# hkust-vgd/scanobjectnn

Hardware: NVIDIA H100
Metric: point-clouds/sec (B=32, N=2048, 15-class) (higher is better)
Workload: dtype f32

## Files before the change

scanobjectnn_b200/csrc/mlp.cu:

```cuda
#include <float.h>

#include "common.cuh"
#include "mlp_internal.cuh"

namespace psa {

constexpr int kMlpThreads = 256;
constexpr int BM = 128;
constexpr int BK = 16;
constexpr int BN_MAX = 128;

__device__ __forceinline__ void cp_async16(void* smem_dst, const void* gmem_src) {
    unsigned d = (unsigned)__cvta_generic_to_shared(smem_dst);
    asm volatile("cp.async.cg.shared.global [%0], [%1], 16;\n" ::"r"(d), "l"(gmem_src));
}
__device__ __forceinline__ void cp_async_commit() { asm volatile("cp.async.commit_group;\n" ::); }
template <int N>
__device__ __forceinline__ void cp_async_wait() {
    asm volatile("cp.async.wait_group %0;\n" ::"n"(N));
}

__device__ __forceinline__ int f2ord(float f) {
    int i = __float_as_int(f);
    return i >= 0 ? i : i ^ 0x7fffffff;
// ... 335 lines not shown
}

template <int TN>
__global__ void __launch_bounds__(kMlpThreads, 2)
dense_layer_kernel(const __grid_constant__ DenseArgs a) {
    constexpr int BN = 16 * TN;
    __shared__ __align__(16) float As[2][BM * LDA_D];
    __shared__ __align__(16) float Ws[2][BK * BN];
    __shared__ int s_pool[(TN == 8) ? 16 * BN : 32 * BN];
    const int tid = threadIdx.x;
    const int ty = tid >> 4, tx = tid & 15;
    const long long row0 = (long long)blockIdx.x * BM;
    const int n0 = blockIdx.y * BN;
    const int K4 = (a.K + 3) & ~3;
    const int nchunks = (K4 + BK - 1) / BK;
    float acc[8][TN];
#pragma unroll
    for (int i = 0; i < 8; ++i)
#pragma unroll
        for (int j = 0; j < TN; ++j) acc[i][j] = 0.f;
    load_a_chunk(As[0], a.x, row0, a.rows, a.K, 0, tid);
    load_w_chunk<BN>(Ws[0], a.W, a.K, a.N, 0, n0, -1, tid);
    cp_async_commit();
    for (int c = 0; c < nchunks; ++c) {
        if (c + 1 < nchunks) {
            load_a_chunk(As[(c + 1) & 1], a.x, row0, a.rows, a.K, (c + 1) * BK, tid);
            load_w_chunk<BN>(Ws[(c + 1) & 1], a.W, a.K, a.N, (c + 1) * BK, n0, -1, tid);
            cp_async_commit();
            cp_async_wait<1>();
        } else {
            cp_async_wait<0>();
        }
        __syncthreads();
        mma_chunk<TN>(As[c & 1], LDA_D, Ws[c & 1], min(BK, K4 - c * BK), acc, ty, tx);
        __syncthreads();
    }
    const int tile_rows = (int)min((long long)BM, a.rows - row0);
    const int pk = a.pool_k;
    if (a.group_add != nullptr) {
#pragma unroll
        for (int i = 0; i < 8; ++i) {
            const int row = ty * 8 + i;
            if (row >= tile_rows) break;
            const float* ga = a.group_add + (row0 + row) / a.group_rows * a.N;
#pragma unroll
            for (int h = 0; h < TN / 4; ++h)
#pragma unroll
                for (int j = 0; j < 4; ++j) {
                    const int col = n0 + h * 64 + tx * 4 + j;
                    if (col < a.N) acc[i][h * 4 + j] += __ldg(ga + col);
                }
        }
    }
    if (pk == 1) {
#pragma unroll
        for (int h = 0; h < TN / 4; ++h) {
            const int col = n0 + h * 64 + tx * 4;
#pragma unroll
            for (int j = 0; j < 4; ++j) {
                if (col + j >= a.N) continue;
                const float sc = a.scale ? __ldg(a.scale + col + j) : 1.f;
                const float sh = a.shift ? __ldg(a.shift + col + j) : 0.f;
#pragma unroll
                for (int i = 0; i < 8; ++i) {
                    const int row = ty * 8 + i;
                    if (row < tile_rows) {
                        float v = fmaf(acc[i][h * 4 + j], sc, sh);
                        if (a.relu) v = fmaxf(v, 0.f);
                        a.out[(row0 + row) * a.N + col + j] = v;
                    }
                }
            }
        }
        return;
    }
    const bool inside = pk <= BM;
    const int ngroups = inside ? (tile_rows / pk) : 1;
    for (int s = tid; s < ngroups * BN; s += kMlpThreads) s_pool[s] = f2ord(__int_as_float(0xff800000));
    __syncthreads();
#pragma unroll
    for (int h = 0; h < TN / 4; ++h) {
        const int col = n0 + h * 64 + tx * 4;
#pragma unroll
        for (int j = 0; j < 4; ++j) {
            if (col + j >= a.N) continue;
            const float sc = a.scale ? __ldg(a.scale + col + j) : 1.f;
            const float sh = a.shift ? __ldg(a.shift + col + j) : 0.f;
            int curg = -1;
            float m = 0.f;
#pragma unroll
            for (int i = 0; i < 8; ++i) {
                const int row = ty * 8 + i;
                if (row >= tile_rows) break;
                float v = fmaf(acc[i][h * 4 + j], sc, sh);
                if (a.relu) v = fmaxf(v, 0.f);
                const int g = inside ? row / pk : 0;
                if (g != curg) {
                    if (curg >= 0) atomicMax(&s_pool[curg * BN + h * 64 + tx * 4 + j], f2ord(m));
                    curg = g;
                    m = v;
                } else {
                    m = fmaxf(m, v);
                }
            }
            if (curg >= 0) atomicMax(&s_pool[curg * BN + h * 64 + tx * 4 + j], f2ord(m));
        }
// ... 199 lines not shown
```

scanobjectnn_b200/csrc/mlp_internal.cuh:

```cuda
#pragma once
#include "common.cuh"

namespace psa {

struct DenseArgs {
    long long rows;
    int K, N;
    int pool_k;
    int relu;
    const float* x;
    const float* W;
    const float* scale;
    const float* shift;
    float* out;
    const float* group_add = nullptr;
    long long group_rows = 0;
};


int launch_dense(const DenseArgs& d, cudaStream_t st);
size_t fc_small_workspace_bytes(int K, int N);
int launch_fc_small(const DenseArgs& d, float* partial, cudaStream_t st);
int sa_module_simt(int b, int n, int m, int c, int nsample, const float* xyz, const float* new_xyz, const float* points,
                   const int* idx, const psa_mlp* mlp, float* out, cudaStream_t st);
int validate_mlp_public(const psa_mlp* mlp, const char* who);
int edgeconv_simt(int b, int n, int c, int k, const float* x, const int* nn_idx, const psa_mlp* mlp, float* out, cudaStream_t st);
int launch_fill_ord_neg_inf(long long total, float* out, cudaStream_t st, const unsigned int* run_if = nullptr);
int launch_decode_ord(long long total, float* out, cudaStream_t st, const unsigned int* run_if = nullptr);
size_t edge_tail_workspace_bytes(int b, int n, int c, int k, int N);
int edge_layer_tail(int b, int n, int c, int k, int N, const float* x, const int* nn_idx, const float* W, const float* PQ, const float* scale,
                    const float* shift, const float* coef, const float* pooled, const float* R, const float* dz, float* dW, float* dx,
                    void* workspace, cudaStream_t st);
int frozen_coef(int N, const float* scale, float* coef, cudaStream_t st);

int mlp_mode();
int tc_np();
int tc_dense_nt(long long rows, int N);
int build_image(int K, int Kp, int N, int Nt, const float* W, uint8_t* image, cudaStream_t st, const unsigned int* run_if = nullptr);
const unsigned int* image_trailer(const uint8_t* image, int Kp, int N);
const float* image_colscale(const uint8_t* image, int Kp, int N);

}

__global__ void edge_wc_kernel(int c, int N, const float* __restrict__ W, float* __restrict__ Wc);
```

scanobjectnn_b200/csrc/tc_mlp.cu:

```cuda
#include <float.h>
#include <stdlib.h>

#include <algorithm>
#include <atomic>
#include <type_traits>

#include "common.cuh"
#include "mlp_internal.cuh"
#include "ring_gemm.cuh"
#include "tc_common.cuh"

namespace psa {

using namespace tc;

constexpr int kMaxTcLayers = 2;


struct TcArgs {
    long long groups;
    int K;
    int n, m;
    const float* xyz;
    const float* new_xyz;
// ... 69 lines not shown
    s_bad[threadIdx.y][threadIdx.x] = bad;
    __syncthreads();
    if (threadIdx.y != 0 || n >= N) return;
    for (int y = 1; y < 8; ++y) { m = fmaxf(m, s_max[y][threadIdx.x]); bad = bad || s_bad[y][threadIdx.x]; }
    int e = 0;
    if (!bad && m > 0.f) e = min(137 - (int)(__float_as_uint(m) >> 23), 64);
    colscale[n] = __int_as_float((127 - e) << 23);
    if (bad) atomicOr(trailer, 1u);
}

template <int NP>
__global__ void tc_prep_weights_kernel(int K, int Kp, int N, int Nt, const float* __restrict__ W, const float* __restrict__ colscale,
                                       uint8_t* __restrict__ image, const unsigned int* __restrict__ run_if) {
    if (run_if != nullptr && *run_if == 0u) return;
    const int KC = Kp / 64;
    const uint32_t bb = tc_block_bytes(Nt, NP), piece = (uint32_t)Nt * 128u;
    uint32_t unused = 0u;
    for (int e = blockIdx.x * blockDim.x + threadIdx.x; e < Kp * N; e += gridDim.x * blockDim.x) {
        const int n = e % N, k = e / N;
        float w = k < K ? __ldg(W + e) : 0.f;
        if (NP == 2) w *= pow2_rcp(__ldg(colscale + n));
        uint32_t pc[NP];
        split_pair<NP>(w, 0.f, pc, unused);
        uint8_t* blk = image + (size_t)((n / Nt) * KC + (k >> 6)) * bb;
        const uint32_t off = swz_off_bf16(n % Nt, k & 63, Nt);
#pragma unroll
        for (int i = 0; i < NP; ++i) *reinterpret_cast<uint16_t*>(blk + i * piece + off) = (uint16_t)(pc[i] & 0xffffu);
    }
}

constexpr int kSaNt = 64;
constexpr int kSaThreads = 256;
constexpr uint32_t kSmemBudget = 220u * 1024u;

struct TcSaLayout {
    uint32_t w[kMaxTcLayers];
    uint32_t ring[2];
    uint32_t ring_bytes;
    uint32_t vec, total;
};

__host__ __device__ inline TcSaLayout tc_sa_layout(const TcArgs& a) {
    TcSaLayout L;
    uint32_t off = 0;
#pragma unroll
    for (int l = 0; l < kMaxTcLayers; ++l) {
        L.w[l] = off;
        if (l < a.nl && !(a.stream_last && l == a.nl - 1)) off += (uint32_t)tc_image_bytes(a.Kd[l], a.Ntot[l], a.np);
    }
    L.ring_bytes = a.stream_last ? (uint32_t)(a.Kd[a.nl - 1] / 64) * tc_block_bytes(kSaNt, a.np) : 0u;
    L.ring[0] = off; off += L.ring_bytes;
    L.ring[1] = off; off += L.ring_bytes;
    L.vec = off;
    off += 8u * a.C1 * 4u;
#pragma unroll
    for (int l = 0; l < kMaxTcLayers; ++l) off += l < a.nl ? 2u * a.Ntot[l] * 4u : 0u;
    L.total = off;
    return L;
}

__host__ __device__ inline int sa_chunk(int K, bool joint) { return (joint ? 128 : 512) / K; }
__host__ __device__ inline uint32_t sa_carry_bytes(const TcArgs& a) { return a.joint ? 0u : 2u * a.Ntot[a.nl - 1] * 4u; }
__host__ __device__ inline uint32_t sa_red_bytes(int chunks) { return 8u * 64u * 4u * (uint32_t)chunks; }

__device__ __forceinline__ void sa_fill_ring(uint32_t q, const uint8_t* image, int ncl, const TcSaLayout& L, uint8_t* base, uint64_t* bars) {
    uint64_t* bar = &bars[q & 1];
    mbar_expect_tx(bar, L.ring_bytes);
    const uint8_t* src = image + (size_t)(q % (uint32_t)ncl) * L.ring_bytes;
    for (uint32_t o = 0; o < L.ring_bytes; o += 32768u) bulk_g2s(base + L.ring[q & 1] + o, src + o, min(32768u, L.ring_bytes - o), bar);
}

template <int NP, int KS, int NCH>
__device__ __forceinline__ void sa_mma_issue(float (&d)[NCH][32], const uint32_t (&A)[NP][8][4], uint32_t wb, uint32_t cstride) {
    constexpr uint32_t bb = tc_block_bytes(kSaNt, NP), piece = kSaNt * 128u;
    wg_fence();
#pragma unroll
    for (int tt = 0; tt < Split<NP>::kTerms; ++tt)
#pragma unroll
        for (int s = 0; s < KS; ++s)
#pragma unroll
            for (int c = 0; c < NCH; ++c)
                wg_mma_rs<NP>(d[c], A[Split<NP>::a(tt)][s][0], A[Split<NP>::a(tt)][s][1], A[Split<NP>::a(tt)][s][2], A[Split<NP>::a(tt)][s][3],
                              wg_desc(wb + (uint32_t)c * cstride + (uint32_t)(s >> 2) * bb + Split<NP>::w(tt) * piece + (uint32_t)(s & 3) * 32u),
                              (tt | s) ? 1u : 0u);
    wg_commit();
}
template <int NP, int KS, int NCH>
__device__ __forceinline__ void sa_mma(float (&d)[NCH][32], const uint32_t (&A)[NP][8][4], uint32_t wb, uint32_t cstride) {
    sa_mma_issue<NP, KS, NCH>(d, A, wb, cstride);
    wg_wait_all();
#pragma unroll
    for (int c = 0; c < NCH; ++c) wg_fence_acc(d[c]);
}

template <int NP, int C1, int NL, int N0>
__global__ void __launch_bounds__(kSaThreads, NP == 2 && C1 == 64 && (NL == 1 || N0 == 64) ? 2 : 1)
tc_sa_kernel(const __grid_constant__ TcArgs a) {
    static_assert((C1 == 64 || C1 == 128) && (NL == 1 || (NL == 2 && (N0 == 64 || N0 == 128))), "unsupported level shape");
    constexpr int last = NL - 1;
    constexpr int KSL = (NL == 2 ? N0 : C1) / 16;
    constexpr bool kDouble = !(C1 == 64 && (NL == 1 || N0 == 64));
    if (a.run_if != nullptr && *a.run_if == 0u) return;
    constexpr uint32_t bb = tc_block_bytes(kSaNt, NP);
    uint32_t ovf = 0u;
    bool ovf_seen = false;
    extern __shared__ uint8_t smem_raw[];
    __shared__ __align__(8) uint64_t s_rbar;
    __shared__ __align__(8) uint64_t s_wbar[2];
    __shared__ unsigned int s_claim[2];
    __shared__ int s_slots[2][2][16];
    __shared__ long long s_desc[2][2][8];

    const int tid = threadIdx.x, lane = tid & 31, warp = tid >> 5;
    const int g = lane >> 2, t = lane & 3;
    uint8_t* base = smem_raw + ((1024u - (smem_u32(smem_raw) & 1023u)) & 1023u);
    const TcSaLayout L = tc_sa_layout(a);

    float* vec = reinterpret_cast<float*>(base + L.vec);
    float* w1x = vec;
    float* w1c = vec + 3 * C1;
    float* s1 = vec + 6 * C1;
    float* t1 = s1 + C1;
    float* sl0 = t1 + C1;
    float* tl0 = sl0 + a.Ntot[0];
    float* slL = NL == 2 ? tl0 + a.Ntot[0] : sl0;
    float* tlL = slL + a.Ntot[last];
    for (int i = tid; i < 3 * C1; i += kSaThreads) {
        const float sc = a.s1 ? __ldg(a.s1 + i % C1) : 1.f;
        w1x[i] = __ldg(a.w1x + i) * sc;
        w1c[i] = a.w1c ? __ldg(a.w1c + i) * sc : 0.f;
    }
    for (int i = tid; i < C1; i += kSaThreads) { s1[i] = a.s1 ? __ldg(a.s1 + i) : 1.f; t1[i] = __ldg(a.t1 + i); }
#pragma unroll
    for (int l = 0; l < NL; ++l)
        for (int i = tid; i < a.Ntot[l]; i += kSaThreads) {
            (l == 0 ? sl0 : slL)[i] = (a.s[l] ? __ldg(a.s[l] + i) : 1.f) * (NP == 2 ? __ldg(a.colscale[l] + i) : 1.f);
            (l == 0 ? tl0 : tlL)[i] = __ldg(a.t[l] + i);
        }
    if (tid == 0) {
        mbar_init(&s_rbar, 1); mbar_init(&s_wbar[0], 1); mbar_init(&s_wbar[1], 1);
        fence_mbar_init();
    }
    __syncthreads();

    const int NCL = a.Ntot[last] / 64;
    uint32_t resident = 0;
#pragma unroll
    for (int l = 0; l < NL; ++l)
        if (!(a.stream_last && l == last)) resident += (uint32_t)tc_image_bytes(a.Kd[l], a.Ntot[l], NP);
    if (tid == 0) {
        if (resident) {
            mbar_expect_tx(&s_rbar, resident);
#pragma unroll
            for (int l = 0; l < NL; ++l) {
                if (a.stream_last && l == last) continue;
                const uint32_t bytes = (uint32_t)tc_image_bytes(a.Kd[l], a.Ntot[l], NP);
                for (uint32_t o = 0; o < bytes; o += 32768u) bulk_g2s(base + L.w[l] + o, a.image[l] + o, min(32768u, bytes - o), &s_rbar);
            }
        }
        if (a.stream_last) { sa_fill_ring(0, a.image[last], NCL, L, base, s_wbar); sa_fill_ring(1, a.image[last], NCL, L, base, s_wbar); }
    }
    if (resident) mbar_wait(&s_rbar, 0);

    const int K = a.K;
    const bool joint = a.joint;
    const int W = joint ? 8 : 4;
    const int C = sa_chunk(K, joint);
    const int unit = joint ? 0 : warp >> 2;
    const int ubar = 1 + unit, uthreads = 32 * W;
    const int ut = joint ? tid : tid & 127, uw0 = joint ? 0 : 4 * unit;
    const int wl = warp - uw0;
    const unsigned nchunks = (unsigned)((a.groups + C - 1) / C);
    float* carry = reinterpret_cast<float*>(base + L.total) + (size_t)unit * a.Ntot[last];
    const int NG = a.pool_chunks, rs = 64 * NG;
    float* red = reinterpret_cast<float*>(base + L.total + sa_carry_bytes(a)) + (size_t)warp * rs;

    auto fill_table = [&](unsigned ch, int b) {
        const long long g0 = (long long)ch * C;
        if (joint) {
            if (ut < C) s_slots[unit][b][ut] = g0 + ut < a.groups ? K / 16 : 0;
            return;
        }
        const long long r0 = g0 * K + wl * 128, rows = a.groups * K;
        int v[4];
#pragma unroll
        for (int q = 0; q < 4; ++q) v[q] = r0 + 32 * q + lane < rows ? __ldg(a.idx + r0 + 32 * q + lane) : 0;
        if (K == 32) {
#pragma unroll
            for (int q = 0; q < 4; ++q) {
                const unsigned d = __ballot_sync(0xffffffffu, v[q] != __shfl_sync(0xffffffffu, v[q], 0));
                const int nb = 4 * wl + q, Ln = d ? 32 - __clz(d) : 1;
                if (lane == 0) s_slots[unit][b][nb] = g0 + nb < a.groups ? (Ln + 15) >> 4 : 0;
            }
        } else {
#pragma unroll
            for (int h = 0; h < 2; ++h) {
                const int f = __shfl_sync(0xffffffffu, v[2 * h], 0);
                const unsigned lo = __ballot_sync(0xffffffffu, v[2 * h] != f), hi = __ballot_sync(0xffffffffu, v[2 * h + 1] != f);
                const int nb = 2 * wl + h, Ln = hi ? 64 - __clz(hi) : lo ? 32 - __clz(lo) : 1;
                if (lane == 0) s_slots[unit][b][nb] = g0 + nb < a.groups ? (Ln + 15) >> 4 : 0;
            }
        }
    };

    constexpr bool kHoldU = NP == 2 && C1 == 128;
    constexpr bool kAhead = NL == 2;
    constexpr int kUH = kHoldU ? C1 / 8 : 1;
    int incl = 0;
    int jn[2];
    long long gn = 0;
    bool carry_next = false;
    float cx = 0.f, cy = 0.f, cz = 0.f, px[2], py[2], pz[2];
    const float* urow[2];
    float2 uh[2][kUH];
    auto gather_a = [&](unsigned ch, int b, int p, int d) {
        if (p == 0) {
            incl = lane < C ? s_slots[unit][b][lane] : 0;
#pragma unroll
            for (int o = 1; o < 16; o <<= 1) {
                const int y = __shfl_up_sync(0xffffffffu, incl, o);
                if (lane >= o) incl += y;
            }
        }
        const int T = __shfl_sync(0xffffffffu, incl, C - 1);
        const int s = p * W + wl, ss = min(s, T - 1);
        const int nb = __popc(__ballot_sync(0xffffffffu, incl <= ss) & ((1u << C) - 1u));
        const int end = __shfl_sync(0xffffffffu, incl, nb), start = nb ? __shfl_sync(0xffffffffu, incl, nb - 1) : 0;
        gn = (long long)ch * C + nb;
        const int row = 16 * (ss - start) + g;
#pragma unroll
        for (int i = 0; i < 2; ++i) jn[i] = __ldg(a.idx + gn * K + row + 8 * i);
        const float* c = a.new_xyz + (size_t)gn * 3;
        cx = __ldg(c); cy = __ldg(c + 1); cz = __ldg(c + 2);
        carry_next = wl == 0 && s < T && s > start;
        if (lane == 0) {
            long long run = 0;
            if (s < T && (wl == 0 || s == start)) {
                const int pe = (p + 1) * W;
                run = gn << 8 | (long long)(min(end, pe) - s) | (s > start ? 16 : 0) | (end > pe ? 32 : 0);
            }
            s_desc[unit][d][wl] = run;
        }
    };
    auto gather_b = [&]() {
        const long long bi = gn / a.m;
#pragma unroll
        for (int i = 0; i < 2; ++i) {
            const float* p = a.xyz + ((size_t)bi * a.n + jn[i]) * 3;
            px[i] = __ldg(p); py[i] = __ldg(p + 1); pz[i] = __ldg(p + 2);
            urow[i] = a.uf ? a.uf + ((size_t)bi * a.n + jn[i]) * C1 : nullptr;
            if constexpr (kHoldU) {
                if (a.uf != nullptr) {
#pragma unroll
                    for (int q = 0; q < kUH; ++q) uh[i][q] = __ldg(reinterpret_cast<const float2*>(urow[i] + 8 * q + 2 * t));
                }
            }
        }
    };

    if (ut == 0) s_claim[unit] = atomicAdd(a.tile_counter, 1u);
    unit_bar_sync(ubar, uthreads);
    unsigned ch = s_claim[unit], claimed = 0;
    if (ch < nchunks) fill_table(ch, 0);
    unit_bar_sync(ubar, uthreads);
    int buf = 0, p = 0;
    if (kAhead && ch < nchunks) { gather_a(ch, 0, 0, 0); gather_b(); }
    uint32_t it = 0;
    for (; ch < nchunks; ++it) {
        if (p == 0 && ut == 0) s_claim[unit] = atomicAdd(a.tile_counter, 1u);
        if (!kAhead) { gather_a(ch, buf, p, it & 1); gather_b(); }

        uint32_t A[NP][8][4];
        {
            float dx[2], dy[2], dz[2];
#pragma unroll
            for (int i = 0; i < 2; ++i) { dx[i] = px[i] - cx; dy[i] = py[i] - cy; dz[i] = pz[i] - cz; }
#pragma unroll
            for (int s = 0; s < C1 / 16; ++s) {
                {
#pragma unroll
                    for (int h = 0; h < 2; ++h) {
                        const int k = 16 * s + 8 * h + 2 * t;
                        const float2 sc = *reinterpret_cast<const float2*>(s1 + k), sh = *reinterpret_cast<const float2*>(t1 + k);
                        const float2 wx = *reinterpret_cast<const float2*>(w1x + k), wy = *reinterpret_cast<const float2*>(w1x + C1 + k),
                                     wz = *reinterpret_cast<const float2*>(w1x + 2 * C1 + k);
#pragma unroll
                        for (int i = 0; i < 2; ++i) {
                            float2 uv;
                            if constexpr (kHoldU) uv = uh[i][2 * s + h];
                            else uv = urow[i] ? __ldg(reinterpret_cast<const float2*>(urow[i] + k)) : sh;
                            float2 v = a.uf ? ffma2_rn(uv, sc, sh) : sh;
                            if (a.w1c != nullptr) {
                                const float2 cwx = *reinterpret_cast<const float2*>(w1c + k), cwy = *reinterpret_cast<const float2*>(w1c + C1 + k),
                                             cwz = *reinterpret_cast<const float2*>(w1c + 2 * C1 + k);
                                v = ffma2_rn(make_float2(cz, cz), cwz, ffma2_rn(make_float2(cy, cy), cwy, ffma2_rn(make_float2(cx, cx), cwx, v)));
                            }
                            v = ffma2_rn(make_float2(dz[i], dz[i]), wz, ffma2_rn(make_float2(dy[i], dy[i]), wy, ffma2_rn(make_float2(dx[i], dx[i]), wx, v)));
                            if (a.relu1) { v.x = fmaxf(v.x, 0.f); v.y = fmaxf(v.y, 0.f); }
                            put_a<NP, 8>(A, s, i + 2 * h, v.x, v.y, ovf);
                        }
                    }
                }
            }
        }

        if constexpr (NL == 2) {
            constexpr int NCH = N0 / 64;
            float d[NCH][32];
            sa_mma<NP, C1 / 16, NCH>(d, A, smem_u32(base + L.w[0]), (uint32_t)(C1 / 64) * bb);
#pragma unroll
            for (int c = 0; c < NCH; ++c) {
#pragma unroll
                for (int jj = 0; jj < 4; ++jj) {
#pragma unroll
                    for (int h = 0; h < 2; ++h) {
                        const int j = 2 * jj + h, col = c * 64 + 8 * j + 2 * t;
                        const float sc0 = sl0[col], sc1 = sl0[col + 1], sh0 = tl0[col], sh1 = tl0[col + 1];
#pragma unroll
                        for (int i = 0; i < 2; ++i) {
                            float v0 = fmaf(d[c][4 * j + 2 * i], sc0, sh0), v1 = fmaf(d[c][4 * j + 2 * i + 1], sc1, sh1);
                            if (a.relu[0]) { v0 = fmaxf(v0, 0.f); v1 = fmaxf(v1, 0.f); }
                            put_a<NP, 8>(A, c * 4 + jj, i + 2 * h, v0, v1, ovf);
                        }
                    }
                }
            }
        }
        if constexpr (NP == 2) { ovf_seen = ovf_seen || f16x2_overflowed(ovf); ovf = 0u; }
        {
            const int N = a.Ntot[last];
            const bool carry_in = carry_next;
            const bool same = (p + 1) * W < __shfl_sync(0xffffffffu, incl, C - 1);
            const bool ahead = kAhead && (same || (p > 0 && claimed < nchunks));
            const bool after_pool = kAhead && !same && p == 0;
            auto issue = [&](float (&acc)[1][32], int nc) {
                uint32_t wb;
                if (a.stream_last) {
                    const uint32_t q = it * (uint32_t)NCL + (uint32_t)nc;
                    mbar_wait(&s_wbar[q & 1], (q >> 1) & 1u);
                    wb = smem_u32(base + L.ring[q & 1]);
                } else {
                    wb = smem_u32(base + L.w[last]) + (uint32_t)(nc * (KSL / 4)) * bb;
                }
                sa_mma_issue<NP, KSL, 1>(acc, A, wb, 0u);
            };
            auto epilogue = [&](float (&acc)[1][32], int nc) {
                wg_fence_acc(acc[0]);
                auto rowmax = [&](int j) {
                    const int col = nc * 64 + 8 * j + 2 * t;
                    const float2 sc = *reinterpret_cast<const float2*>(slL + col), sh = *reinterpret_cast<const float2*>(tlL + col);
                    float lo0 = fmaf(acc[0][4 * j], sc.x, sh.x), hi0 = fmaf(acc[0][4 * j + 2], sc.x, sh.x);
                    float lo1 = fmaf(acc[0][4 * j + 1], sc.y, sh.y), hi1 = fmaf(acc[0][4 * j + 3], sc.y, sh.y);
                    if (a.relu[last]) { lo0 = fmaxf(lo0, 0.f); hi0 = fmaxf(hi0, 0.f); lo1 = fmaxf(lo1, 0.f); hi1 = fmaxf(hi1, 0.f); }
                    return make_float2(fmaxf(lo0, hi0), fmaxf(lo1, hi1));
                };
                float v[8];
                const bool up = (g >> 2) & 1;
#pragma unroll
                for (int j = 0; j < 4; ++j) {
                    const float2 lo = rowmax(j), hi = rowmax(j + 4);
                    v[2 * j] = fmaxf(up ? hi.x : lo.x, __shfl_xor_sync(0xffffffffu, up ? lo.x : hi.x, 16));
                    v[2 * j + 1] = fmaxf(up ? hi.y : lo.y, __shfl_xor_sync(0xffffffffu, up ? lo.y : hi.y, 16));
                }
                colmax_halve<4>(v, (g >> 1) & 1);
                colmax_halve<2>(v, g & 1);
                float2 m = make_float2(v[0], v[1]);
                const int x = 8 * g + 2 * t;
                float* dst = red + (nc % NG) * 64 + x;
                {
                    const float2 c = *reinterpret_cast<const float2*>(carry_in ? carry + nc * 64 + x : dst);
                    m.x = carry_in ? fmaxf(m.x, c.x) : m.x;
                    m.y = carry_in ? fmaxf(m.y, c.y) : m.y;
                }
                *reinterpret_cast<float2*>(dst) = m;
            };
            auto pool = [&](int gi) {
                unit_bar_sync(ubar, uthreads);
                if (gi == 0 && p == 0) {
                    claimed = s_claim[unit];
                    if (claimed < nchunks) fill_table(claimed, buf ^ 1);
                }
                if (a.stream_last && tid == 0)
                    sa_fill_ring(it * (uint32_t)NCL + (uint32_t)gi + 2u, a.image[last], NCL, L, base, s_wbar);
                const long long run = s_desc[unit][it & 1][wl];
                const int len = (int)(run & 15);
                if (len != 0) {
                    for (int c = 0; c < NG; ++c) {
                        const float2* r = reinterpret_cast<const float2*>(red + c * 64) + lane;
                        float2 mx = r[0];
#pragma unroll
                        for (int w = 1; w < 8; ++w)
                            if (w < len) { const float2 v = r[w * rs / 2]; mx.x = fmaxf(mx.x, v.x); mx.y = fmaxf(mx.y, v.y); }
                        const int col = (gi * NG + c) * 64 + 2 * lane;
                        if (run & 32) *reinterpret_cast<float2*>(carry + col) = mx;
                        else *reinterpret_cast<float2*>(a.out + (size_t)(run >> 8) * N + col) = mx;
                    }
                }
                unit_bar_sync(ubar, uthreads);
                if (gi == 0 && after_pool && claimed < nchunks) { gather_a(claimed, buf ^ 1, 0, (it + 1) & 1); gather_b(); }
            };
            float d0[1][32];
            for (int c0 = 0; c0 < NCL; c0 += NG) {
                const int end = c0 + NG;
                issue(d0, c0);
                if (ahead && c0 == 0) gather_a(same ? ch : claimed, same ? buf : buf ^ 1, same ? p + 1 : 0, (it + 1) & 1);
                if constexpr (kDouble) {
                    float d1[1][32];
                    int nc = c0;
                    for (; nc + 2 < end; nc += 2) {
                        issue(d1, nc + 1); wg_wait<1>(); epilogue(d0, nc);
                        issue(d0, nc + 2); wg_wait<1>(); epilogue(d1, nc + 1);
                    }
                    if (nc + 1 < end) {
                        issue(d1, nc + 1); wg_wait<1>(); epilogue(d0, nc);
                        if (ahead && nc + 2 == NCL) gather_b();
                        wg_wait<0>(); epilogue(d1, nc + 1);
                    } else {
                        if (ahead && nc + 1 == NCL) gather_b();
                        wg_wait<0>(); epilogue(d0, nc);
                    }
                } else {
                    for (int nc = c0;;) {
                        if (ahead && nc + 1 == NCL) gather_b();
                        wg_wait<0>(); epilogue(d0, nc);
                        if (++nc == end) break;
                        issue(d0, nc);
                    }
                }
                pool(c0 / NG);
            }
            if (!same) { ch = claimed; buf ^= 1; p = 0; }
            else ++p;
        }
    }
    if constexpr (NP == 2) {
        if (ovf_seen) atomicOr(a.ovf, 1u);
        if (tid == 0)
            for (int l = 0; l < NL; ++l)
                if (a.wflag[l] != nullptr && *a.wflag[l] != 0u) atomicOr(a.ovf, 1u);
    }
    if (tid == 0 && a.stream_last)
        for (uint32_t q = it * (uint32_t)NCL; q < it * (uint32_t)NCL + 2u; ++q) mbar_wait(&s_wbar[q & 1], (q >> 1) & 1u);
}

struct TcDenseArgs {
    long long rows;
    int K, Kp, N;
    int pool_k;
    int relu;
    const float* x;
    const float* scale;
    const float* shift;
    const float* xyz3;
    const float* w3;
    float* out;
    const float* in_scale = nullptr;
    const float* in_shift = nullptr;
    int in_relu = 0;
    float* stat_partial = nullptr;
    const float* group_add = nullptr;
    long long group_rows = 0;
    RingArgs ring;
};

template <int NP, int NC>
struct DenseOp {
    static constexpr int Nt = 64 * NC;
    const TcDenseArgs& a;
    static constexpr bool kClaim = true;
    static constexpr uint32_t kBudget = 210u * 1024u;
    struct Smem {
        float red[2][8][Nt];
        __align__(16) float aff[2][3][Nt];
    };
    struct Unit {
        int nb, col0, par;
// ... 224 lines not shown
    return reinterpret_cast<const unsigned int*>(image + tc_image_trailer_off(Kp, N, 2));
}
const float* image_colscale(const uint8_t* image, int Kp, int N) {
    return reinterpret_cast<const float*>(image + tc_image_colscale_off(Kp, N, 2));
}

static long long tc_dense_units(long long rows, int N, int Nt) { return (rows + 127) / 128 * (N / Nt); }

struct StepWords {
    unsigned int* flag;
    unsigned int* counters;
};
static StepWords step_words(unsigned int* region, int l) { return {region + l, region + PSA_MAX_MLP_LAYERS + 2 * l}; }
constexpr int kClusterFlagStep = 3;

struct DenseStep {
    long long rows;
    int K, N, pool_k, relu;
    const float* x;
    const float* W;
    const float* scale;
    const float* shift;
    float* out;
    const float* xyz3 = nullptr;
    const float* w3 = nullptr;
    const float* group_add = nullptr;
    long long group_rows = 0;
    const uint8_t* prebuilt = nullptr;
    uint8_t* img = nullptr;
    StepWords words{};
    float* fc_partial = nullptr;
};

static bool dense_on_tc(long long rows, int K, int N, int pool_k) { return g_mlp_mode != 1 && tc_dense_eligible(rows, K, N, pool_k); }

static TcDenseArgs tc_dense_args(const DenseStep& s) {
    TcDenseArgs a;
    a.rows = s.rows; a.K = s.K; a.Kp = (s.K + 63) & ~63; a.N = s.N; a.pool_k = s.pool_k; a.relu = s.relu;
    a.x = s.x; a.scale = s.scale; a.shift = s.shift; a.out = s.out; a.xyz3 = s.xyz3; a.w3 = s.w3;
    a.group_add = s.group_add; a.group_rows = s.group_rows;
    return a;
}
static RingWeights tc_dense_weights(const DenseStep& s) {
    return RingWeights{s.K, (s.K + 63) & ~63, s.N, tc_dense_nt(s.rows, s.N) & ~kImageFlags, s.W, s.img, s.img + tc_dense_image_off3(s.K, s.N), s.prebuilt};
}

static int run_dense(const DenseStep& s, cudaStream_t st) {
    if (dense_on_tc(s.rows, s.K, s.N, s.pool_k)) {
        RingPool pool;
        if (s.pool_k > 128) { pool.out = s.out; pool.count = s.rows / s.pool_k * s.N; }
        const RingWeights w = tc_dense_weights(s);
        return ring_run(kDenseRing, tc_dense_args(s), tc_dense_units(s.rows, s.N, w.Nt), w, s.words.flag, s.words.counters, st, pool);
    }
    PSA_SUPPORTED(s.xyz3 == nullptr, "sa_group_all: layer 0 must run on the tensor-core path");
    DenseArgs d;
    d.rows = s.rows; d.K = s.K; d.N = s.N; d.pool_k = s.pool_k; d.relu = s.relu;
    d.x = s.x; d.W = s.W; d.scale = s.scale; d.shift = s.shift; d.out = s.out;
    d.group_add = s.group_add; d.group_rows = s.group_rows;
    if (s.fc_partial != nullptr && s.rows <= 32 && s.pool_k == 1 && s.group_add == nullptr) return launch_fc_small(d, s.fc_partial, st);
    return launch_dense(d, st);
}

bool tc_train_fwd_eligible(long long rows, int K, int N) {
    return rows >= 128 && K >= 128 && K <= 512 && N >= 128 && (N % 128) == 0;
}
int launch_tc_dense_train(long long rows, int K, int N, const float* x, const float* in_scale, const float* in_shift, int in_relu,
                          const float* W, const float* bias, float* y, float* stat_partial, uint8_t* image_ws, cudaStream_t st) {
    const int Kp = (K + 63) & ~63;
    int rc = build_image(K, Kp, N, 128 | kImageBf16x3, W, image_ws, st);
    if (rc != PSA_OK) return rc;
    TcDenseArgs a;
    a.rows = rows; a.K = K; a.Kp = Kp; a.N = N; a.pool_k = 1; a.relu = 0;
    a.x = x; a.scale = nullptr; a.shift = bias; a.out = y; a.xyz3 = nullptr; a.w3 = nullptr;
    a.in_scale = in_scale; a.in_shift = in_shift; a.in_relu = in_relu; a.stat_partial = stat_partial;
    a.ring.image = image_ws;
    return ring_launch(kDenseRing, 3, 128, &a, tc_dense_units(rows, N, 128), st);
}

static const uint8_t* prebuilt_image(const psa_mlp* mlp, int l, int row0, int Nt) {
    if (mlp->image[l] != nullptr && mlp->image_nt[l] == Nt && mlp->image_row0[l] == row0) return reinterpret_cast<const uint8_t*>(mlp->image[l]);
    return nullptr;
}

bool tc_sa_eligible(const psa_mlp* mlp, int c, int nsample, TcArgs* out, int np) {
    if (mlp->n_layers < 2 || mlp->n_layers > 1 + kMaxTcLayers) return false;
    if (!(nsample == 32 || nsample == 64 || nsample == 128)) return false;
    if (mlp->channels[0] != 3 + c) return false;
    const int C1 = mlp->channels[1];
    if (!(C1 == 64 || C1 == 128)) return false;
    TcArgs a{};
    a.C1 = C1;
    a.nl = mlp->n_layers - 1;
    a.np = np;
    for (int l = 0; l < a.nl; ++l) {
        a.Kd[l] = mlp->channels[1 + l];
        a.Ntot[l] = mlp->channels[2 + l];
        if (!(a.Kd[l] == 64 || a.Kd[l] == 128)) return false;
        const bool is_last = (l == a.nl - 1);
        if (!is_last && !(a.Ntot[l] == 64 || a.Ntot[l] == 128)) return false;
        if (is_last && !(a.Ntot[l] == 64 || a.Ntot[l] % 128 == 0)) return false;
    }
    a.stream_last = 0;
    if (tc_sa_layout(a).total + 1024 > kSmemBudget) a.stream_last = 1;
    if (tc_sa_layout(a).total + 1024 > kSmemBudget) return false;
    *out = a;
    return true;
}
bool tc_sa_eligible(const psa_mlp* mlp, int c, int nsample, TcArgs* out) {
    TcArgs a3;
    if (!tc_sa_eligible(mlp, c, nsample, &a3, 3)) return false;
    if (g_tc_np == 3) { *out = a3; return true; }
    return tc_sa_eligible(mlp, c, nsample, out, 2);
// ... 8 lines not shown

static int tc_sa_image_nt() { return kSaNt | image_flag(g_tc_np); }

template <int NP, int C1, int NL, int N0>
static int launch_tc_sa_shape(const TcArgs& a, long long ctas_needed, size_t smem, cudaStream_t st) {
    PSA_CUDA(cudaFuncSetAttribute(tc_sa_kernel<NP, C1, NL, N0>, cudaFuncAttributeMaxDynamicSharedMemorySize, (int)smem));
    int dev = 0, sms = 0, per_sm = 0;
    PSA_CUDA(cudaGetDevice(&dev));
    PSA_CUDA(cudaDeviceGetAttribute(&sms, cudaDevAttrMultiProcessorCount, dev));
    PSA_CUDA(cudaOccupancyMaxActiveBlocksPerMultiprocessor(&per_sm, tc_sa_kernel<NP, C1, NL, N0>, kSaThreads, smem));
    const long long resident = (long long)sms * (per_sm > 0 ? per_sm : 1);
    const int ctas = (int)(ctas_needed < 1 ? 1 : ctas_needed < resident ? ctas_needed : resident);
    tc_sa_kernel<NP, C1, NL, N0><<<ctas, kSaThreads, smem, st>>>(a);
    return check_launch("tc_sa_kernel");
}

template <int NP>
static int launch_tc_sa_np(TcArgs& a, cudaStream_t st) {
    const uint32_t limit = 223u * 1024u;
    a.joint = a.K == 128 || a.stream_last;
    if (!a.joint && tc_sa_layout(a).total + 1024 + sa_carry_bytes(a) + sa_red_bytes(1) > limit) a.joint = 1;
    const size_t used = (size_t)tc_sa_layout(a).total + 1024 + sa_carry_bytes(a);
    const int ncl = a.Ntot[a.nl - 1] / 64;
    a.pool_chunks = 1;
    if (!a.stream_last)
        for (int ng = ncl; ng > 1; --ng)
            if (ncl % ng == 0 && used + sa_red_bytes(ng) <= limit) { a.pool_chunks = ng; break; }
    const int C = sa_chunk(a.K, a.joint);
    const long long nchunks = (a.groups + C - 1) / C;
    const long long ctas_needed = a.joint ? nchunks : (nchunks + 1) / 2;
    const size_t smem = used + sa_red_bytes(a.pool_chunks);
    if (a.nl == 1) return a.C1 == 64 ? launch_tc_sa_shape<NP, 64, 1, 0>(a, ctas_needed, smem, st) : launch_tc_sa_shape<NP, 128, 1, 0>(a, ctas_needed, smem, st);
    if (a.C1 == 64) return a.Ntot[0] == 64 ? launch_tc_sa_shape<NP, 64, 2, 64>(a, ctas_needed, smem, st) : launch_tc_sa_shape<NP, 64, 2, 128>(a, ctas_needed, smem, st);
    return a.Ntot[0] == 64 ? launch_tc_sa_shape<NP, 128, 2, 64>(a, ctas_needed, smem, st) : launch_tc_sa_shape<NP, 128, 2, 128>(a, ctas_needed, smem, st);
}

static int tc_sa_run(TcArgs& a, int b, int n, int m, int c, int nsample, const float* xyz, const float* new_xyz, const float* points,
                     const int* idx, const psa_mlp* mlp, const float* w1c, float* out, void* workspace, cudaStream_t st) {
    int rc = PSA_OK;
    uint8_t* ws = reinterpret_cast<uint8_t*>(workspace);
    unsigned int* region = reinterpret_cast<unsigned int*>(ws);
    const StepWords words = step_words(region, 1);
    PSA_CUDA(cudaMemsetAsync(ws, 0, 256, st));
    ws += 256;
    RingWeights w[kMaxTcLayers];
    for (int l = 0; l < a.nl; ++l) {
        const int K = a.Kd[l], N = a.Ntot[l];
        w[l] = RingWeights{K, K, N, kSaNt, mlp->weight[1 + l], ws, ws + tc_image_alloc_bytes(K, N, 2), prebuilt_image(mlp, 1 + l, 0, tc_sa_image_nt())};
        ws += tc_image_alloc_bytes(K, N, 2) + tc_image_alloc_bytes(K, N, 3);
    }
    const float* uf = nullptr;
    if (c > 0) {
        const long long rows = (long long)b * n;
        DenseStep u{rows, c, a.C1, 1, 0, points, mlp->weight[0] + (size_t)3 * a.C1, nullptr, nullptr, reinterpret_cast<float*>(ws)};
        u.prebuilt = prebuilt_image(mlp, 0, 3, tc_dense_nt(rows, a.C1));
        u.img = ws + (((size_t)rows * a.C1 * sizeof(float) + 255) & ~(size_t)255);
        u.words = step_words(region, 0);
        if ((rc = run_dense(u, st)) != PSA_OK) return rc;
        uf = u.out;
    }
    auto fill = [&](TcArgs& t) {
        t.groups = (long long)b * m; t.K = nsample; t.n = n; t.m = m;
        t.xyz = xyz; t.new_xyz = new_xyz; t.idx = idx; t.out = out; t.uf = uf;
        t.w1x = mlp->weight[0]; t.s1 = mlp->scale[0]; t.t1 = mlp->shift[0]; t.relu1 = mlp->relu[0];
        t.ovf = nullptr; t.run_if = nullptr; t.w1c = w1c;
        for (int l = 0; l < t.nl; ++l) {
            t.s[l] = mlp->scale[1 + l]; t.t[l] = mlp->shift[1 + l]; t.relu[l] = mlp->relu[1 + l]; t.wflag[l] = nullptr; t.colscale[l] = nullptr;
        }
    };
    fill(a);
    for (int l = 0; l < a.nl; ++l) {
        if ((rc = ring_image(w[l], a.np, nullptr, st, a.image[l])) != PSA_OK) return rc;
        if (a.np == 2) { a.wflag[l] = image_trailer(a.image[l], w[l].Kp, w[l].N); a.colscale[l] = image_colscale(a.image[l], w[l].Kp, w[l].N); }
    }
    a.tile_counter = words.counters;
    if (a.np == 3) return launch_tc_sa_np<3>(a, st);
    a.ovf = words.flag;
    rc = launch_tc_sa_np<2>(a, st);
    if (rc != PSA_OK) return rc;
    TcArgs a3;
    PSA_REQUIRE(tc_sa_eligible(mlp, c, nsample, &a3, 3), "sa_module: internal error (bf16x3 eligibility)");
    fill(a3);
    for (int l = 0; l < a3.nl; ++l)
        if ((rc = ring_image(w[l], 3, words.flag, st, a3.image[l])) != PSA_OK) return rc;
    a3.tile_counter = words.counters + 1;
    a3.run_if = words.flag;
    return launch_tc_sa_np<3>(a3, st);
}

struct TcGroupAllArgs {
    int c;
    int N[3];
    int Nt[3];
    const float* points;
    const float* xyz;
    const float* w3;
    const uint8_t* image[3];
    const float* colscale[3];
    const unsigned int* wflag[3];
    const float* scale[3];
    const float* shift[3];
    int relu[3];
    float* out;
    unsigned int* ovf;
};

constexpr int kGaStages = 3;
// ... 688 lines not shown
```

Before: 95930.

## Fold xyz term and BN scale/shift of first SA layer into precomputed per-point features

The per-point dense precompute now adds the xyz·W contribution and applies the first layer's scale and shift, so the grouped SA kernel only adds a per-centroid correction (center times a combined weight) and applies ReLU. This removes the per-neighbor xyz loads and the several FMAs per channel from the hot gather loop, and drops the s1 shared-memory vector. The SIMT dense fallback gains an xyz3/w3 path, and optional clock64 timestamp instrumentation is added behind a compile flag. Register-held U is now restricted to the two-layer case, and the rewritten algebra may change rounding slightly.

```diff
diff --git a/scanobjectnn_b200/csrc/mlp.cu b/scanobjectnn_b200/csrc/mlp.cu
--- a/scanobjectnn_b200/csrc/mlp.cu
+++ b/scanobjectnn_b200/csrc/mlp.cu
@@ -411,6 +411,23 @@
                 }
         }
     }
+    if (a.xyz3 != nullptr) {
+#pragma unroll
+        for (int i = 0; i < 8; ++i) {
+            const int row = ty * 8 + i;
+            if (row >= tile_rows) break;
+            const float* q = a.xyz3 + (row0 + row) * 3;
+            const float x0 = __ldg(q), x1 = __ldg(q + 1), x2 = __ldg(q + 2);
+#pragma unroll
+            for (int h = 0; h < TN / 4; ++h)
+#pragma unroll
+                for (int j = 0; j < 4; ++j) {
+                    const int col = n0 + h * 64 + tx * 4 + j;
+                    if (col < a.N)
+                        acc[i][h * 4 + j] = fmaf(x2, __ldg(a.w3 + 2 * a.N + col), fmaf(x1, __ldg(a.w3 + a.N + col), fmaf(x0, __ldg(a.w3 + col), acc[i][h * 4 + j])));
+                }
+        }
+    }
     if (pk == 1) {
 #pragma unroll
         for (int h = 0; h < TN / 4; ++h) {
diff --git a/scanobjectnn_b200/csrc/mlp_internal.cuh b/scanobjectnn_b200/csrc/mlp_internal.cuh
--- a/scanobjectnn_b200/csrc/mlp_internal.cuh
+++ b/scanobjectnn_b200/csrc/mlp_internal.cuh
@@ -15,6 +15,8 @@
     float* out;
     const float* group_add = nullptr;
     long long group_rows = 0;
+    const float* xyz3 = nullptr;
+    const float* w3 = nullptr;
 };
 
 
diff --git a/scanobjectnn_b200/csrc/tc_mlp.cu b/scanobjectnn_b200/csrc/tc_mlp.cu
--- a/scanobjectnn_b200/csrc/tc_mlp.cu
+++ b/scanobjectnn_b200/csrc/tc_mlp.cu
@@ -145,7 +145,7 @@
     L.ring[0] = off; off += L.ring_bytes;
     L.ring[1] = off; off += L.ring_bytes;
     L.vec = off;
-    off += 8u * a.C1 * 4u;
+    off += 7u * a.C1 * 4u;
 #pragma unroll
     for (int l = 0; l < kMaxTcLayers; ++l) off += l < a.nl ? 2u * a.Ntot[l] * 4u : 0u;
     L.total = off;
@@ -185,6 +185,40 @@
 #pragma unroll
     for (int c = 0; c < NCH; ++c) wg_fence_acc(d[c]);
 }
+
+#ifdef PSA_SA_STAMPS
+enum SaStamp { kSaTop, kSaInputs, kSaLayer1, kSaL2Issued, kSaL2Retired, kSaL2Epi, kSaPool1, kSaPool2, kSaNextA, kSaNextB, kSaChunk0 };
+constexpr int kSaStampCtas = 264, kSaStampPasses = 64, kSaStampPhases = kSaChunk0 + 3 * 4;
+__device__ long long g_sa_stamps[kSaStampCtas][2][kSaStampPasses][kSaStampPhases];
+extern "C" PSA_API int psa_sa_stamps(long long* dst) {
+    return cudaMemcpyFromSymbol(dst, g_sa_stamps, sizeof(g_sa_stamps)) == cudaSuccess ? 0 : 1;
+}
+extern "C" PSA_API int psa_sa_stamps_clear(void) {
+    void* p = nullptr;
+    if (cudaGetSymbolAddress(&p, g_sa_stamps) != cudaSuccess) return 1;
+    return cudaMemset(p, 0, sizeof(g_sa_stamps)) == cudaSuccess ? 0 : 1;
+}
+#define SA_STAMP(p, k)                                                                                              \
+    do {                                                                                                            \
+        if ((threadIdx.x & 127) == 0 && blockIdx.x < kSaStampCtas && (p) < kSaStampPasses && (k) < kSaStampPhases) \
+            g_sa_stamps[blockIdx.x][threadIdx.x >> 7][(p)][(k)] = clock64();                                        \
+    } while (0)
+#define SA_STAMP_AFTER(p, k, r)                                                                                     \
+    do {                                                                                                            \
+        if ((threadIdx.x & 127) == 0 && blockIdx.x < kSaStampCtas && (p) < kSaStampPasses) {                        \
+            volatile long long* p_ = &g_sa_stamps[blockIdx.x][threadIdx.x >> 7][(p)][(k)];                          \
+            *p_ = (long long)__float_as_uint(__fmul_rn((r), 0.f));                                                  \
+            *p_ = clock64();                                                                                        \
+        }                                                                                                           \
+    } while (0)
+#else
+#define SA_STAMP(p, k) \
+    do {               \
+    } while (0)
+#define SA_STAMP_AFTER(p, k, r) \
+    do {                        \
+    } while (0)
+#endif
 
 template <int NP, int C1, int NL, int N0>
 __global__ void __launch_bounds__(kSaThreads, NP == 2 && C1 == 64 && (NL == 1 || N0 == 64) ? 2 : 1)
@@ -212,8 +246,7 @@
     float* vec = reinterpret_cast<float*>(base + L.vec);
     float* w1x = vec;
     float* w1c = vec + 3 * C1;
-    float* s1 = vec + 6 * C1;
-    float* t1 = s1 + C1;
+    float* t1 = vec + 6 * C1;
     float* sl0 = t1 + C1;
     float* tl0 = sl0 + a.Ntot[0];
     float* slL = NL == 2 ? tl0 + a.Ntot[0] : sl0;
@@ -221,9 +254,9 @@
     for (int i = tid; i < 3 * C1; i += kSaThreads) {
         const float sc = a.s1 ? __ldg(a.s1 + i % C1) : 1.f;
         w1x[i] = __ldg(a.w1x + i) * sc;
-        w1c[i] = a.w1c ? __ldg(a.w1c + i) * sc : 0.f;
-    }
-    for (int i = tid; i < C1; i += kSaThreads) { s1[i] = a.s1 ? __ldg(a.s1 + i) : 1.f; t1[i] = __ldg(a.t1 + i); }
+        w1c[i] = (a.w1c ? __ldg(a.w1c + i) : 0.f) * sc - (a.uf ? w1x[i] : 0.f);
+    }
+    for (int i = tid; i < C1; i += kSaThreads) t1[i] = __ldg(a.t1 + i);
 #pragma unroll
     for (int l = 0; l < NL; ++l)
         for (int i = tid; i < a.Ntot[l]; i += kSaThreads) {
@@ -296,8 +329,8 @@
         }
     };
 
-    constexpr bool kHoldU = NP == 2 && C1 == 128;
     constexpr bool kAhead = NL == 2;
+    constexpr bool kHoldU = NP == 2 && C1 == 128 && kAhead;
     constexpr int kUH = kHoldU ? C1 / 8 : 1;
     int incl = 0;
     int jn[2];
@@ -339,8 +372,10 @@
         const long long bi = gn / a.m;
 #pragma unroll
         for (int i = 0; i < 2; ++i) {
-            const float* p = a.xyz + ((size_t)bi * a.n + jn[i]) * 3;
-            px[i] = __ldg(p); py[i] = __ldg(p + 1); pz[i] = __ldg(p + 2);
+            if (a.uf == nullptr) {
+                const float* p = a.xyz + ((size_t)bi * a.n + jn[i]) * 3;
+                px[i] = __ldg(p); py[i] = __ldg(p + 1); pz[i] = __ldg(p + 2);
+            }
             urow[i] = a.uf ? a.uf + ((size_t)bi * a.n + jn[i]) * C1 : nullptr;
             if constexpr (kHoldU) {
                 if (a.uf != nullptr) {
@@ -361,46 +396,69 @@
     uint32_t it = 0;
     for (; ch < nchunks; ++it) {
         if (p == 0 && ut == 0) s_claim[unit] = atomicAdd(a.tile_counter, 1u);
+        SA_STAMP(it, kSaTop);
         if (!kAhead) { gather_a(ch, buf, p, it & 1); gather_b(); }
+        SA_STAMP_AFTER(it, kSaInputs, a.uf == nullptr ? px[0] : kHoldU ? uh[0][0].x : __ldg(urow[0] + 2 * t));
 
         uint32_t A[NP][8][4];
-        {
+        if (a.uf != nullptr) {
+#pragma unroll
+            for (int s = 0; s < C1 / 16; ++s) {
+#pragma unroll
+                for (int h = 0; h < 2; ++h) {
+                    const int k = 16 * s + 8 * h + 2 * t;
+                    const float2 cwx = *reinterpret_cast<const float2*>(w1c + k), cwy = *reinterpret_cast<const float2*>(w1c + C1 + k),
+                                 cwz = *reinterpret_cast<const float2*>(w1c + 2 * C1 + k);
+                    const float2 ct = ffma2_rn(make_float2(cz, cz), cwz, ffma2_rn(make_float2(cy, cy), cwy, fmul2_rn(make_float2(cx, cx), cwx)));
+#pragma unroll
+                    for (int i = 0; i < 2; ++i) {
+                        float2 v;
+                        if constexpr (kHoldU) v = uh[i][2 * s + h];
+                        else v = __ldg(reinterpret_cast<const float2*>(urow[i] + k));
+                        v = fadd2_rn(v, ct);
+                        if (a.relu1) { v.x = fmaxf(v.x, 0.f); v.y = fmaxf(v.y, 0.f); }
+                        put_a<NP, 8>(A, s, i + 2 * h, v.x, v.y, ovf);
+                    }
+                }
+            }
+        } else {
             float dx[2], dy[2], dz[2];
 #pragma unroll
             for (int i = 0; i < 2; ++i) { dx[i] = px[i] - cx; dy[i] = py[i] - cy; dz[i] = pz[i] - cz; }
 #pragma unroll
             for (int s = 0; s < C1 / 16; ++s) {
-                {
-#pragma unroll
-                    for (int h = 0; h < 2; ++h) {
-                        const int k = 16 * s + 8 * h + 2 * t;
-                        const float2 sc = *reinterpret_cast<const float2*>(s1 + k), sh = *reinterpret_cast<const float2*>(t1 + k);
-                        const float2 wx = *reinterpret_cast<const float2*>(w1x + k), wy = *reinterpret_cast<const float2*>(w1x + C1 + k),
-                                     wz = *reinterpret_cast<const float2*>(w1x + 2 * C1 + k);
-#pragma unroll
-                        for (int i = 0; i < 2; ++i) {
-                            float2 uv;
-                            if constexpr (kHoldU) uv = uh[i][2 * s + h];
-                            else uv = urow[i] ? __ldg(reinterpret_cast<const float2*>(urow[i] + k)) : sh;
-                            float2 v = a.uf ? ffma2_rn(uv, sc, sh) : sh;
-                            if (a.w1c != nullptr) {
-                                const float2 cwx = *reinterpret_cast<const float2*>(w1c + k), cwy = *reinterpret_cast<const float2*>(w1c + C1 + k),
-                                             cwz = *reinterpret_cast<const float2*>(w1c + 2 * C1 + k);
-                                v = ffma2_rn(make_float2(cz, cz), cwz, ffma2_rn(make_float2(cy, cy), cwy, ffma2_rn(make_float2(cx, cx), cwx, v)));
-                            }
-                            v = ffma2_rn(make_float2(dz[i], dz[i]), wz, ffma2_rn(make_float2(dy[i], dy[i]), wy, ffma2_rn(make_float2(dx[i], dx[i]), wx, v)));
-                            if (a.relu1) { v.x = fmaxf(v.x, 0.f); v.y = fmaxf(v.y, 0.f); }
-                            put_a<NP, 8>(A, s, i + 2 * h, v.x, v.y, ovf);
+#pragma unroll
+                for (int h = 0; h < 2; ++h) {
+                    const int k = 16 * s + 8 * h + 2 * t;
+                    const float2 sh = *reinterpret_cast<const float2*>(t1 + k);
+                    const float2 wx = *reinterpret_cast<const float2*>(w1x + k), wy = *reinterpret_cast<const float2*>(w1x + C1 + k),
+                                 wz = *reinterpret_cast<const float2*>(w1x + 2 * C1 + k);
+#pragma unroll
+                    for (int i = 0; i < 2; ++i) {
+                        float2 v = sh;
+                        if (a.w1c != nullptr) {
+                            const float2 cwx = *reinterpret_cast<const float2*>(w1c + k), cwy = *reinterpret_cast<const float2*>(w1c + C1 + k),
+                                         cwz = *reinterpret_cast<const float2*>(w1c + 2 * C1 + k);
+                            v = ffma2_rn(make_float2(cz, cz), cwz, ffma2_rn(make_float2(cy, cy), cwy, ffma2_rn(make_float2(cx, cx), cwx, v)));
                         }
+                        v = ffma2_rn(make_float2(dz[i], dz[i]), wz, ffma2_rn(make_float2(dy[i], dy[i]), wy, ffma2_rn(make_float2(dx[i], dx[i]), wx, v)));
+                        if (a.relu1) { v.x = fmaxf(v.x, 0.f); v.y = fmaxf(v.y, 0.f); }
+                        put_a<NP, 8>(A, s, i + 2 * h, v.x, v.y, ovf);
                     }
                 }
             }
         }
+        SA_STAMP(it, kSaLayer1);
 
         if constexpr (NL == 2) {
             constexpr int NCH = N0 / 64;
             float d[NCH][32];
-            sa_mma<NP, C1 / 16, NCH>(d, A, smem_u32(base + L.w[0]), (uint32_t)(C1 / 64) * bb);
+            sa_mma_issue<NP, C1 / 16, NCH>(d, A, smem_u32(base + L.w[0]), (uint32_t)(C1 / 64) * bb);
+            SA_STAMP(it, kSaL2Issued);
+            wg_wait_all();
+#pragma unroll
+            for (int c = 0; c < NCH; ++c) wg_fence_acc(d[c]);
+            SA_STAMP(it, kSaL2Retired);
 #pragma unroll
             for (int c = 0; c < NCH; ++c) {
 #pragma unroll
@@ -418,6 +476,7 @@
                     }
                 }
             }
+            SA_STAMP(it, kSaL2Epi);
         }
         if constexpr (NP == 2) { ovf_seen = ovf_seen || f16x2_overflowed(ovf); ovf = 0u; }
         {
@@ -436,9 +495,11 @@
                     wb = smem_u32(base + L.w[last]) + (uint32_t)(nc * (KSL / 4)) * bb;
                 }
                 sa_mma_issue<NP, KSL, 1>(acc, A, wb, 0u);
+                SA_STAMP(it, kSaChunk0 + 3 * nc);
             };
             auto epilogue = [&](float (&acc)[1][32], int nc) {
                 wg_fence_acc(acc[0]);
+                SA_STAMP(it, kSaChunk0 + 3 * nc + 1);
                 auto rowmax = [&](int j) {
                     const int col = nc * 64 + 8 * j + 2 * t;
                     const float2 sc = *reinterpret_cast<const float2*>(slL + col), sh = *reinterpret_cast<const float2*>(tlL + col);
@@ -466,9 +527,11 @@
                     m.y = carry_in ? fmaxf(m.y, c.y) : m.y;
                 }
                 *reinterpret_cast<float2*>(dst) = m;
+                SA_STAMP(it, kSaChunk0 + 3 * nc + 2);
             };
             auto pool = [&](int gi) {
                 unit_bar_sync(ubar, uthreads);
+                SA_STAMP(it, kSaPool1);
                 if (gi == 0 && p == 0) {
                     claimed = s_claim[unit];
                     if (claimed < nchunks) fill_table(claimed, buf ^ 1);
@@ -490,13 +553,22 @@
                     }
                 }
                 unit_bar_sync(ubar, uthreads);
-                if (gi == 0 && after_pool && claimed < nchunks) { gather_a(claimed, buf ^ 1, 0, (it + 1) & 1); gather_b(); }
+                SA_STAMP(it, kSaPool2);
+                if (gi == 0 && after_pool && claimed < nchunks) {
+                    gather_a(claimed, buf ^ 1, 0, (it + 1) & 1);
+                    SA_STAMP(it, kSaNextA);
+                    gather_b();
+                    SA_STAMP(it, kSaNextB);
+                }
             };
             float d0[1][32];
             for (int c0 = 0; c0 < NCL; c0 += NG) {
                 const int end = c0 + NG;
                 issue(d0, c0);
-                if (ahead && c0 == 0) gather_a(same ? ch : claimed, same ? buf : buf ^ 1, same ? p + 1 : 0, (it + 1) & 1);
+                if (ahead && c0 == 0) {
+                    gather_a(same ? ch : claimed, same ? buf : buf ^ 1, same ? p + 1 : 0, (it + 1) & 1);
+                    SA_STAMP(it, kSaNextA);
+                }
                 if constexpr (kDouble) {
                     float d1[1][32];
                     int nc = c0;
@@ -506,15 +578,15 @@
                     }
                     if (nc + 1 < end) {
                         issue(d1, nc + 1); wg_wait<1>(); epilogue(d0, nc);
-                        if (ahead && nc + 2 == NCL) gather_b();
+                        if (ahead && nc + 2 == NCL) { gather_b(); SA_STAMP(it, kSaNextB); }
                         wg_wait<0>(); epilogue(d1, nc + 1);
                     } else {
-                        if (ahead && nc + 1 == NCL) gather_b();
+                        if (ahead && nc + 1 == NCL) { gather_b(); SA_STAMP(it, kSaNextB); }
                         wg_wait<0>(); epilogue(d0, nc);
                     }
                 } else {
                     for (int nc = c0;;) {
-                        if (ahead && nc + 1 == NCL) gather_b();
+                        if (ahead && nc + 1 == NCL) { gather_b(); SA_STAMP(it, kSaNextB); }
                         wg_wait<0>(); epilogue(d0, nc);
                         if (++nc == end) break;
                         issue(d0, nc);
@@ -845,12 +917,11 @@
         const RingWeights w = tc_dense_weights(s);
         return ring_run(kDenseRing, tc_dense_args(s), tc_dense_units(s.rows, s.N, w.Nt), w, s.words.flag, s.words.counters, st, pool);
     }
-    PSA_SUPPORTED(s.xyz3 == nullptr, "sa_group_all: layer 0 must run on the tensor-core path");
     DenseArgs d;
     d.rows = s.rows; d.K = s.K; d.N = s.N; d.pool_k = s.pool_k; d.relu = s.relu;
     d.x = s.x; d.W = s.W; d.scale = s.scale; d.shift = s.shift; d.out = s.out;
-    d.group_add = s.group_add; d.group_rows = s.group_rows;
-    if (s.fc_partial != nullptr && s.rows <= 32 && s.pool_k == 1 && s.group_add == nullptr) return launch_fc_small(d, s.fc_partial, st);
+    d.group_add = s.group_add; d.group_rows = s.group_rows; d.xyz3 = s.xyz3; d.w3 = s.w3;
+    if (s.fc_partial != nullptr && s.rows <= 32 && s.pool_k == 1 && s.group_add == nullptr && s.xyz3 == nullptr) return launch_fc_small(d, s.fc_partial, st);
     return launch_dense(d, st);
 }
 
@@ -965,7 +1036,9 @@
     const float* uf = nullptr;
     if (c > 0) {
         const long long rows = (long long)b * n;
-        DenseStep u{rows, c, a.C1, 1, 0, points, mlp->weight[0] + (size_t)3 * a.C1, nullptr, nullptr, reinterpret_cast<float*>(ws)};
+        DenseStep u{rows, c, a.C1, 1, 0, points, mlp->weight[0] + (size_t)3 * a.C1, mlp->scale[0], mlp->shift[0], reinterpret_cast<float*>(ws)};
+        u.xyz3 = xyz;
+        u.w3 = mlp->weight[0];
         u.prebuilt = prebuilt_image(mlp, 0, 3, tc_dense_nt(rows, a.C1));
         u.img = ws + (((size_t)rows * a.C1 * sizeof(float) + 255) & ~(size_t)255);
         u.words = step_words(region, 0);
```

Result: faster. 101,000, median of 6 (+5.3%).
